# baegwangbin/MaGNet

Hardware: NVIDIA H100
Metric: frames/sec (640x480, 4 views, 64 hyp) (higher is better)
Workload: dtype f32

## Files before the change

### magnet_b200/csrc/api.cu

```cuda
#include <atomic>
#include <cstdlib>
#include <cstdio>
#include <cstring>

#include "common.cuh"

namespace magnet {
cudaError_t launch_cost_direct(const CostParams& p, int depth_mode, int src_layout, int C, bool cw,
                               bool softmax, cudaStream_t st, int* launches);
cudaError_t launch_cost_cells(const CostParams& p, int mode, int C, bool cw, bool reuse, cudaStream_t st);
cudaError_t launch_softmax_planes(float* vol, int B, int D, int HW, cudaStream_t st);
bool cells_supports(int C, int D, int layout);
cudaError_t launch_cost_tma(const CostParams& p, int mode, int C, bool cw, cudaStream_t st);
bool tma_supports(int C, int D, int V, int layout);
void tma_launch_info(int B, int H, int W, int D, int* grid, int* block, int* smem);
cudaError_t launch_cost_mma(const CostParams& p, int mode, bool cw, cudaStream_t st);
bool mma_supports(int C, int D, int V, int layout);
void mma_launch_info(int B, int H, int W, int D, int* grid, int* block, int* smem);
size_t split16_buffer_bytes(int N, int H, int W);
cudaError_t launch_repack_split16(const float* src, const float* gmm, void* dst, int N, int C, int H, int W,
                                  cudaStream_t st, int* launches);
#ifdef MAGNET_MMA_DEBUG
void mma_set_debug_buffer(float* p);
#endif
cudaError_t launch_repack_pixc(const float* src, const float* gmm, float* dst, int N, int C, int H, int W,
                               cudaStream_t st);
void cells_launch_info(int B, int H, int W, int D, int* grid, int* block, int* smem);
cudaError_t launch_pack_cameras(const float* intM, const float* R, int64_t r_sb, int64_t r_sv, int64_t r_si,
                                int64_t r_sj, const float* t, int64_t t_sb, int64_t t_sv, int64_t t_si,
                                const int32_t* is_valid, int B, int V, magnet_camera* out, cudaStream_t st);
cudaError_t launch_repack(const float* src, float* dst, int N, int C, int H, int W, cudaStream_t st);
cudaError_t launch_sample(const float* gmm, const float* k_host, int B, int D, int HW, float* dvol,
                          cudaStream_t st);
cudaError_t launch_update_fwd(const float* dout, const float* gmm0, int B, int HW, float* out, cudaStream_t st);
cudaError_t launch_update_bwd(const float* gout, const float* dout, const float* gmm0, int B, int HW, float* gin,
                              cudaStream_t st);
cudaError_t launch_relative_poses(const float* ext_ref, const float* ext_nghbr, int B, int V, float* poses,
                                  int32_t* valid, cudaStream_t st);
cudaError_t launch_camera_rays(const double* raw, int B, int H, int W, float* intM, float* rays, cudaStream_t st);
cudaError_t launch_upsample_fwd(const float* depth, const float* mask, int B, int CH, int H, int W, int k, float* out,
                                cudaStream_t st);
cudaError_t launch_upsample_bwd(const float* gout, const float* depth, const float* mask, int B, int CH, int H, int W,
                                int k, float* gdepth, float* gmask, cudaStream_t st);
cudaError_t launch_cost_f_bwd(const BwdParams& p, cudaStream_t st, int* launches);
cudaError_t launch_cost_f_bwd_mma(const BwdParams& p, cudaStream_t st, int* launches);
bool f_bwd_mma_supports(int C, int V);
cudaError_t launch_cost_cw_bwd(const CwBwdParams& p, const CwBwdParams* split, int C, int mode, bool mask_mma,
                               const float* grad_out, cudaStream_t st, int* launches);
bool cw_bwd_supports(int C);
#ifdef MAGNET_MMA_DEBUG
void f_bwd_mma_set_debug_buffer(float* p);
#endif
int fnet_l1_partials(int B, int HW);
cudaError_t launch_fnet_l1_fwd(const float* scores, const float* planes, const float* gt, const uint8_t* mask, int B,
                               int D, int HW, float* partial, cudaStream_t st);
cudaError_t launch_fnet_l1_bwd(const float* scores, const float* planes, const float* gt, const uint8_t* mask,
                               float scale, const float* grad_scale, int B, int D, int HW, float* grad_scores,
                               cudaStream_t st);
cudaError_t launch_upsample_nll_fwd(const float* depth, const float* mask, const float* gt, const uint8_t* gtm, int B,
                                    int H, int W, int k, float* partial, cudaStream_t st);
cudaError_t launch_upsample_nll_bwd(const float* depth, const float* mask, const float* gt, const uint8_t* gtm, float scale,
                                    int B, int H, int W, int k, float* gdepth, float* gmask, cudaStream_t st);
}

namespace {
std::atomic<uint64_t> g_launches{0};
thread_local char g_cuda_err[256] = "";

int cuda_fail(cudaError_t e) {
  snprintf(g_cuda_err, sizeof(g_cuda_err), "%s: %s", cudaGetErrorName(e), cudaGetErrorString(e));
  return MAGNET_ERR_CUDA;
}

int validate_cost(const magnet_cost_args* a) {
  if (!a) return MAGNET_ERR_NULL;
// ... 222 lines not shown
                            const int32_t* is_valid, int32_t B, int32_t V, magnet_camera* cams_out,
                            void* stream) {
  if (!intM || !R || !t || !is_valid || !cams_out) return MAGNET_ERR_NULL;
  if (B <= 0 || V <= 0) return MAGNET_ERR_SHAPE;
  cudaError_t e = magnet::launch_pack_cameras(intM, R, r_sb, r_sv, r_si, r_sj, t, t_sb, t_sv, t_si, is_valid, B, V,
                                              cams_out, (cudaStream_t)stream);
  if (e != cudaSuccess) return cuda_fail(e);
  g_launches += 1;
  return MAGNET_OK;
}

int magnet_repack_tiled32_f32(const float* src_nchw, float* dst, int32_t N, int32_t C, int32_t H, int32_t W,
                            void* stream) {
  if (!src_nchw || !dst) return MAGNET_ERR_NULL;
  if (N <= 0 || C <= 0 || H <= 0 || W <= 0) return MAGNET_ERR_SHAPE;
  if (C % 4 != 0 || C / 4 > 65535 || N > 65535) return MAGNET_ERR_UNSUPPORTED;
  if (reinterpret_cast<uintptr_t>(dst) % 16 != 0) return MAGNET_ERR_ALIGN;
  cudaError_t e = magnet::launch_repack(src_nchw, dst, N, C, H, W, (cudaStream_t)stream);
  if (e != cudaSuccess) return cuda_fail(e);
  g_launches += 1;
  return MAGNET_OK;
}

int magnet_repack_pixc_f32(const float* src_nchw, const float* src_gmm, float* dst, int32_t N, int32_t C, int32_t H,
                           int32_t W, void* stream) {
  if (!src_nchw || !dst) return MAGNET_ERR_NULL;
  if (N <= 0 || C <= 0 || H <= 0 || W <= 0 || N > 65535) return MAGNET_ERR_SHAPE;
  if (C != 16 && C != 32 && C != 64) return MAGNET_ERR_UNSUPPORTED;
  if (reinterpret_cast<uintptr_t>(dst) % 16 != 0) return MAGNET_ERR_ALIGN;
  cudaError_t e = magnet::launch_repack_pixc(src_nchw, src_gmm, dst, N, C, H, W, (cudaStream_t)stream);
  if (e != cudaSuccess) return cuda_fail(e);
  g_launches += 1;
  return MAGNET_OK;
}

size_t magnet_split16_bytes(int32_t N, int32_t H, int32_t W) {
  if (N <= 0 || H <= 0 || W <= 0) return 0;
  return magnet::split16_buffer_bytes(N, H, W);
}

int magnet_repack_split16_f32(const float* src_nchw, const float* src_gmm, void* dst, int32_t N, int32_t C, int32_t H,
                              int32_t W, void* stream) {
  if (!src_nchw || !dst) return MAGNET_ERR_NULL;
  if (N <= 0 || C <= 0 || H <= 0 || W <= 0 || N > 65535) return MAGNET_ERR_SHAPE;
  if (C != 64) return MAGNET_ERR_UNSUPPORTED;
  if (reinterpret_cast<uintptr_t>(dst) % 16 != 0 || reinterpret_cast<uintptr_t>(src_nchw) % 16 != 0) return MAGNET_ERR_ALIGN;
  int launches = 0;
  cudaError_t e = magnet::launch_repack_split16(src_nchw, src_gmm, dst, N, C, H, W, (cudaStream_t)stream, &launches);
  if (e != cudaSuccess) return cuda_fail(e);
  g_launches += launches;
  return MAGNET_OK;
}

#ifdef MAGNET_MMA_DEBUG
void magnet_mma_debug_buffer(float* p) { magnet::mma_set_debug_buffer(p); }
void magnet_f_bwd_mma_debug_buffer(float* p) { magnet::f_bwd_mma_set_debug_buffer(p); }
#endif

int magnet_sample_depths_f32(const float* gmm, const float* k_host, int32_t B, int32_t D, int32_t HW,
                             float* d_volume, void* stream) {
  if (!gmm || !k_host || !d_volume) return MAGNET_ERR_NULL;
  if (B <= 0 || D <= 0 || HW <= 0) return MAGNET_ERR_SHAPE;
  if (D > MAGNET_MAX_PLANES || B > 65535) return MAGNET_ERR_UNSUPPORTED;
  cudaError_t e = magnet::launch_sample(gmm, k_host, B, D, HW, d_volume, (cudaStream_t)stream);
  if (e != cudaSuccess) return cuda_fail(e);
  g_launches += 1;
  return MAGNET_OK;
}

int magnet_gaussian_update_fwd_f32(const float* d_output, const float* ref_gmm, int32_t B, int32_t HW,
                                   float* out, void* stream) {
  if (!d_output || !ref_gmm || !out) return MAGNET_ERR_NULL;
  if (B <= 0 || HW <= 0 || B > 65535) return MAGNET_ERR_SHAPE;
  cudaError_t e = magnet::launch_update_fwd(d_output, ref_gmm, B, HW, out, (cudaStream_t)stream);
  if (e != cudaSuccess) return cuda_fail(e);
  g_launches += 1;
  return MAGNET_OK;
}

int magnet_gaussian_update_bwd_f32(const float* grad_out, const float* d_output, const float* ref_gmm,
                                   int32_t B, int32_t HW, float* grad_d_output, void* stream) {
  if (!grad_out || !d_output || !ref_gmm || !grad_d_output) return MAGNET_ERR_NULL;
  if (B <= 0 || HW <= 0 || B > 65535) return MAGNET_ERR_SHAPE;
  cudaError_t e = magnet::launch_update_bwd(grad_out, d_output, ref_gmm, B, HW, grad_d_output, (cudaStream_t)stream);
  if (e != cudaSuccess) return cuda_fail(e);
  g_launches += 1;
  return MAGNET_OK;
}

int magnet_relative_poses_f32(const float* ext_ref, const float* ext_nghbr, int32_t B, int32_t V, float* poses_out,
                              int32_t* is_valid_out, void* stream) {
  if (!ext_ref || !ext_nghbr || !poses_out || !is_valid_out) return MAGNET_ERR_NULL;
  if (B <= 0 || V <= 0) return MAGNET_ERR_SHAPE;
  cudaError_t e = magnet::launch_relative_poses(ext_ref, ext_nghbr, B, V, poses_out, is_valid_out, (cudaStream_t)stream);
  if (e != cudaSuccess) return cuda_fail(e);
  g_launches += 1;
  return MAGNET_OK;
}

int magnet_camera_rays_f32(const double* raw_intrinsics, int32_t B, int32_t H, int32_t W, float* intM_out,
                           float* rays_out, void* stream) {
  if (!raw_intrinsics || !intM_out || !rays_out) return MAGNET_ERR_NULL;
  if (B <= 0 || H <= 0 || W <= 0 || B > 65535) return MAGNET_ERR_SHAPE;
  cudaError_t e = magnet::launch_camera_rays(raw_intrinsics, B, H, W, intM_out, rays_out, (cudaStream_t)stream);
  if (e != cudaSuccess) return cuda_fail(e);
  g_launches += 1;
  return MAGNET_OK;
}
// ... 94 lines not shown
```

### magnet_b200/csrc/cost_mma.cu

```cuda
#include <cuda_fp16.h>

#include <algorithm>
#include <atomic>
#include <cstddef>
#include <mutex>
#include <type_traits>

#include "common.cuh"
#include "tma_common.cuh"
#include "cw_mask.cuh"

namespace magnet {

constexpr int MNT = 256;
constexpr int MTW = 8, MTH = 8;
constexpr int MPX = MTW * MTH;
constexpr int MCH = 64;
constexpr int MSEG = 32;
constexpr int MMAXV = 16;
constexpr int SEG_BYTES = 2048;
constexpr int META_SEG_BYTES = 128;

constexpr int MOFF_A = 0;
constexpr int MOFF_R = 16384;
constexpr int MR_BYTES = 67584;
constexpr int MOFF_META = MOFF_R + MR_BYTES;
constexpr int MOFF_CAM = MOFF_META + MSEG * META_SEG_BYTES;
constexpr int MOFF_KS = MOFF_CAM + MMAXV * 64;
constexpr int MOFF_BBOX = MOFF_KS + MCH * 4;
constexpr int MOFF_BAR = MOFF_BBOX + 64;
constexpr int MOFF_ACC = MOFF_BAR + 64;
constexpr int MOFF_PIX = MOFF_ACC + MCH * 65 * 4;
constexpr int M_SMEM_USED = MOFF_PIX + 8 * 8 * 32;
constexpr int M_SMEM_TOTAL = M_SMEM_USED + 1024;
static_assert(MR_BYTES >= MSEG * SEG_BYTES && MR_BYTES >= MPX * 264 * 4 && MR_BYTES >= MCH * 65 * 4, "region R");
static_assert(2 * (M_SMEM_TOTAL + 1024) <= 227 * 1024, "two CTAs per SM");

__host__ __device__ inline size_t split16_bytes(size_t N, size_t H, size_t W) {
  return SPLIT16_HEADER + N * H * W * 256 + N * H * (W + 1) * 16;
}

constexpr int MMA_SLOTS = 1024;
__device__ unsigned g_mma_next[MMA_SLOTS];
__device__ unsigned g_mma_done[MMA_SLOTS];

__device__ __forceinline__ float lds_f32(uint32_t a) {
  float v;
  asm volatile("ld.shared.f32 %0, [%1];" : "=f"(v) : "r"(a));
  return v;
}
__device__ __forceinline__ float4 lds_f32x4(uint32_t a) {
  float4 v;
  asm volatile("ld.shared.v4.f32 {%0, %1, %2, %3}, [%4];" : "=f"(v.x), "=f"(v.y), "=f"(v.z), "=f"(v.w) : "r"(a));
  return v;
}
template <int MODE, bool CW>
__global__ void __launch_bounds__(MNT, 2)
cost_mma_kernel(const __grid_constant__ CostParams p, const __grid_constant__ CUtensorMap tm_ref,
                const __grid_constant__ CUtensorMap tm_src, const __grid_constant__ CUtensorMap tm_meta, const int nchunks,
                const int n_items, const int slot, float* __restrict__ dbg) {
  extern __shared__ unsigned char smem_raw[];
  const uint32_t raw = smem_u32(smem_raw);
  const uint32_t padb = (1024u - (raw & 1023u)) & 1023u;
  unsigned char* smem = smem_raw + padb;
  const uint32_t sbase = raw + padb;
  const magnet_camera* cams_s = reinterpret_cast<const magnet_camera*>(smem + MOFF_CAM);
  float* ks = reinterpret_cast<float*>(smem + MOFF_KS);
  int* bbox = reinterpret_cast<int*>(smem + MOFF_BBOX);
  float* regR = reinterpret_cast<float*>(smem + MOFF_R);
  const uint32_t bar_tma = sbase + MOFF_BAR, bar_cam = sbase + MOFF_BAR + 24;
  float* acc_s = reinterpret_cast<float*>(smem + MOFF_ACC);
  const unsigned FULL = 0xffffffffu;

  const int tid = threadIdx.x, lane = tid & 31, warp = tid >> 5;
  const int H = p.H, W = p.W, HW = p.HW, D = p.D, V = p.V;
  const int tiles_x = (W + MTW - 1) / MTW;
  const int items_per_b = tiles_x * ((H + MTH - 1) / MTH) * nchunks;

  const unsigned char* refbuf = reinterpret_cast<const unsigned char*>(p.ref_feat);
  const unsigned char* srcbuf = reinterpret_cast<const unsigned char*>(p.src_feat);
  const Split16Header* hdr_ref = reinterpret_cast<const Split16Header*>(refbuf);
  const Split16Header* hdr_src = reinterpret_cast<const Split16Header*>(srcbuf);
  volatile int* next_item = reinterpret_cast<volatile int*>(smem + MOFF_BAR + 40);

  if (tid == 0) {
    mbar_init(bar_tma, 1);
    mbar_init(bar_cam, 1);
    fence_mbar_init();
    prefetch_tmap(&tm_ref);
    prefetch_tmap(&tm_src);
    prefetch_tmap(&tm_meta);
  }
  if (tid < 8) bbox[tid] = (tid & 1) ? -(1 << 28) : (1 << 28);
  __syncthreads();
  uint32_t ph_tma = 0, ph_cam = 0;
  int it = 0;
  int cur_b = -1;
  const float xmax = (float)W + 1.0f, ymax = (float)H + 1.0f;
  const float kappa = p.kappa;
  const uint32_t g_row0 = sbase + MOFF_R, m_base = sbase + MOFF_META;

  int item = blockIdx.x;
  while (item < n_items) {
  const int b = item / items_per_b;
  const int rem = item - b * items_per_b;
  const int tile = rem / nchunks;
  const int jc = (rem - tile * nchunks) * MCH;
  const int Dc = min(MCH, D - jc);
  const int tx0 = (tile % tiles_x) * MTW, ty0 = (tile / tiles_x) * MTH;

  if (tid == 0) {
    if (b != cur_b) {
      mbar_arrive_expect_tx(bar_cam, (uint32_t)V * 64u);
      bulk_load(sbase + MOFF_CAM, p.cams + (size_t)b * V, (uint32_t)V * 64u, bar_cam);
    }
    tma_load_5d(sbase + MOFF_A, &tm_ref, bar_tma, 0, tx0, ty0, 0, b);
    *next_item = (int)gridDim.x + (int)atomicAdd(&g_mma_next[slot], 1u);
  }
  if (tid < MCH) ks[tid] = MODE != MAGNET_DEPTH_VOLUME ? p.k[min(jc + tid, D - 1)] : 0.0f;
  for (int idx = tid; idx < MCH * 65; idx += MNT) acc_s[idx] = 0.0f;
  __syncthreads();

  const int py = ty0 + warp;
  float R0, R1, R2, MU = 0.f, SG = 0.f;
  unsigned livemask;
  {
    const int px = tx0 + (lane & 7);
    const bool live = px < W && py < H;
    const int n = min(py, H - 1) * W + min(px, W - 1);
    R0 = ldg_f(p.rays + ((size_t)b * 3 + 0) * HW + n);
    R1 = ldg_f(p.rays + ((size_t)b * 3 + 1) * HW + n);
    R2 = ldg_f(p.rays + ((size_t)b * 3 + 2) * HW + n);
    if (MODE == MAGNET_DEPTH_GAUSS) {
      MU = ldg_f(p.ref_gmm + ((size_t)b * 2 + 0) * HW + n);
      SG = ldg_f(p.ref_gmm + ((size_t)b * 2 + 1) * HW + n);
    }
    livemask = __ballot_sync(FULL, live) & 0xffu;
  }
  float2 dvol[MODE == MAGNET_DEPTH_VOLUME ? MTW : 1];
  float2 k2 = make_float2(0.f, 0.f);
  if (MODE == MAGNET_DEPTH_VOLUME) {
    for (int idx = tid; idx < MCH * MPX; idx += MNT) {
      const int j = idx >> 6, pp = idx & 63;
      const int y = ty0 + (pp >> 3), x = tx0 + (pp & 7);
      const size_t n = (size_t)min(y, H - 1) * W + min(x, W - 1);
      regR[j * 65 + pp] = ldg_f(p.d_volume + ((size_t)b * D + jc + min(j, Dc - 1)) * HW + n);
    }
    __syncthreads();
#pragma unroll
    for (int i = 0; i < MTW; ++i) dvol[i] = make_float2(regR[lane * 65 + warp * 8 + i], regR[(lane + 32) * 65 + warp * 8 + i]);
    fence_proxy_async();
    __syncthreads();
  } else {
    k2 = make_float2(ks[lane], ks[lane + 32]);
  }
  auto depth2 = [&](const int i, const float mu, const float sg) -> float2 {
    if (MODE == MAGNET_DEPTH_VOLUME) return dvol[i];
    if (MODE == MAGNET_DEPTH_PLANES) return k2;
    return fadd2_rn(make_float2(mu, mu), make_float2(__fmul_rn(sg, k2.x), __fmul_rn(sg, k2.y)));
  };
  float4* pixt = reinterpret_cast<float4*>(smem + MOFF_PIX) + warp * 16;

  if (b != cur_b) {
    mbar_wait_or_trap(bar_cam, ph_cam);
    ph_cam ^= 1u;
    cur_b = b;
  }
  bool first = true;

  for (int v = 0; v < V; ++v) {
    const magnet_camera* cam = cams_s + v;
    if (cam->valid != 1.0f) continue;
    const float a0 = cam->a[0], a1 = cam->a[1], a2 = cam->a[2];
    const float Q0 = __fmaf_rn(cam->A[2], R2, __fmaf_rn(cam->A[1], R1, __fmul_rn(cam->A[0], R0)));
    const float Q1 = __fmaf_rn(cam->A[5], R2, __fmaf_rn(cam->A[4], R1, __fmul_rn(cam->A[3], R0)));
    const float Q2 = __fmaf_rn(cam->A[8], R2, __fmaf_rn(cam->A[7], R1, __fmul_rn(cam->A[6], R0)));
    __syncwarp();
    if (lane < 8) {
      pixt[2 * lane] = make_float4(Q0, Q1, Q2, 0.0f);
      pixt[2 * lane + 1] = make_float4(Q2, MU, SG, 0.0f);
    }
    __syncwarp();
    const int vb = v * p.B + b;
    auto project_px = [&](const int i, float2& ix, float2& iy, float2& z) {
      const float4 t1 = pixt[2 * i], t2 = pixt[2 * i + 1];
      project2(depth2(i, t2.y, t2.z), a0, a1, a2, t1.x, t1.y, t1.z, ix, iy, z);
      ix.x = clamp_coord(ix.x, xmax); ix.y = clamp_coord(ix.y, xmax);
      iy.x = clamp_coord(iy.x, ymax); iy.y = clamp_coord(iy.y, ymax);
    };

    float xl = 1e9f, xh = -1e9f, yl = 1e9f, yh = -1e9f;
#pragma unroll
    for (int i = 0; i < MTW; ++i) {
      float2 ix, iy, z;
      project_px(i, ix, iy, z);
      if ((livemask >> i) & 1u) {
        xl = fminf(xl, fminf(ix.x, ix.y)); xh = fmaxf(xh, fmaxf(ix.x, ix.y));
        yl = fminf(yl, fminf(iy.x, iy.y)); yh = fmaxf(yh, fmaxf(iy.x, iy.y));
      }
    }
    int* bb = bbox + (it & 1) * 4;
    {
      const int r0 = __reduce_min_sync(FULL, (int)floorf(xl)), r1 = __reduce_max_sync(FULL, (int)floorf(xh));
      const int r2 = __reduce_min_sync(FULL, (int)floorf(yl)), r3 = __reduce_max_sync(FULL, (int)floorf(yh));
      if (lane == 0) { atomicMin(bb + 0, r0); atomicMax(bb + 1, r1); atomicMin(bb + 2, r2); atomicMax(bb + 3, r3); }
    }
    fence_proxy_async();
    __syncthreads();
    const int wx0 = bb[0], wx1 = bb[1], wy0 = bb[2], wy1 = bb[3];
    if (tid < 4) bbox[((it + 1) & 1) * 4 + tid] = (tid & 1) ? -(1 << 28) : (1 << 28);
    ++it;
    const int nseg_all = (wx1 - wx0 + 2 + 7) >> 3, rows_all = wy1 - wy0 + 2;
    const int nsw = min(nseg_all, 16);
    const int rmax = nseg_all * rows_all <= MSEG ? rows_all : max(2, MSEG / nsw);
    const int stepx = 8 * nsw - 1, stepy = rmax - 1;

    for (int sy = wy0; sy <= wy1; sy += stepy) {
      const int rows = min(stepy, wy1 - sy + 1) + 1;
      for (int sx = wx0; sx <= wx1; sx += stepx) {
        const int nseg = (min(stepx, wx1 - sx + 1) + 1 + 7) >> 3;
        const int nsegs = nseg * rows;
        if (tid == 0)
          mbar_arrive_expect_tx(bar_tma, (uint32_t)nsegs * (SEG_BYTES + (CW ? META_SEG_BYTES : 0)) + (first ? 16384u : 0u));
        first = false;
        if (lane == 0) {
          for (int s = warp; s < nsegs; s += MNT / 32) {
            const int r = s / nseg, xb = s - r * nseg;
            tma_load_5d(sbase + MOFF_R + (uint32_t)s * SEG_BYTES, &tm_src, bar_tma, 0, sx + 8 * xb, sy + r, 0, vb);
            if (CW) tma_load_4d(m_base + (uint32_t)s * META_SEG_BYTES, &tm_meta, bar_tma, 0, sx + 8 * xb + 1, sy + r, vb);
          }
        }
        __syncwarp();
        const int npad = (nsegs * 8 + 15) & ~15;
        const int gp = ((npad + 23) & ~31) + 8;
        mbar_wait_or_trap(bar_tma, ph_tma);
        ph_tma ^= 1u;
        {
          const int wg = warp >> 2;
          float acc[64];
#pragma unroll
          for (int e = 0; e < 64; ++e) acc[e] = 0.0f;
          const uint32_t bseg = sbase + MOFF_R + (uint32_t)(wg * 16 * SEG_BYTES);
          const uint64_t a_hi = gmma_desc_sw128(sbase + MOFF_A, 1024), a_lo = gmma_desc_sw128(sbase + MOFF_A + 8192, 1024);
          const uint64_t b_hi = gmma_desc_sw128(bseg, SEG_BYTES), b_lo = gmma_desc_sw128(bseg + 1024, SEG_BYTES);
          __syncwarp();
          if (wg == 0 || npad > 128) {
            wgmma_fence();
#pragma unroll
            for (int pr = 0; pr < 3; ++pr) {
              const uint64_t ad = pr == 0 ? a_lo : a_hi, bd = pr == 1 ? b_lo : b_hi;
#pragma unroll
              for (int kk = 0; kk < 4; ++kk) wgmma_m64n128k16_f16(acc, ad + 2u * kk, bd + 2u * kk, (pr | kk) != 0);
            }
            wgmma_commit();
            wgmma_wait_all();
          }
          __syncthreads();
          const int r0 = ((warp & 3) << 4) + (lane >> 2);
          float* g0 = regR + (size_t)r0 * gp + wg * 128 + 2 * (lane & 3);
#pragma unroll
          for (int j = 0; j < 16; ++j) {
            if (wg * 128 + 8 * j < npad) {
              *reinterpret_cast<float2*>(g0 + 8 * j) = make_float2(acc[4 * j], acc[4 * j + 1]);
              *reinterpret_cast<float2*>(g0 + 8 * gp + 8 * j) = make_float2(acc[4 * j + 2], acc[4 * j + 3]);
            }
          }
          __syncthreads();
        }
#ifdef MAGNET_MMA_DEBUG
        if (dbg != nullptr && item == 0 && v == 0 && sy == wy0 && sx == wx0) {
          if (tid == 0) {
            dbg[0] = (float)sx; dbg[1] = (float)sy; dbg[2] = (float)nseg; dbg[3] = (float)rows; dbg[4] = (float)npad;
            dbg[5] = (float)gp; dbg[6] = (float)v; dbg[7] = 3.0f; dbg[8] = hdr_ref->scale; dbg[9] = hdr_src->scale;
          }
          for (int idx = tid; idx < MPX * npad; idx += MNT) dbg[16 + (idx / npad) * 256 + idx % npad] = regR[(idx / npad) * gp + idx % npad];
        }
#endif
        const bool single = nseg_all * rows_all <= MSEG;
        auto phase_c = [&](auto single_tag) {
          constexpr bool SINGLE = decltype(single_tag)::value;
          const float MAGIC = 12582912.0f;
          const float sxf = (float)sx, syf = (float)sy;
          const float xend = sx + stepx > wx1 ? 1e9f : (float)(sx + stepx), yend = sy + stepy > wy1 ? 1e9f : (float)(sy + stepy);
          const float pitch4f = (float)(nseg * 32);
          const float c0f = MAGIC - 4.0f * sxf - pitch4f * syf;
          const uint32_t pitch4 = (uint32_t)nseg * 32u;
          uint32_t rowaddr = g_row0 + (uint32_t)(warp * 8 * gp) * 4u;
          float* accp = acc_s + lane * 65 + warp * 8;
#pragma unroll
          for (int i = 0; i < MTW; ++i, rowaddr += (uint32_t)gp * 4u) {
            if (!((livemask >> i) & 1u)) continue;
            float2 x, y, z;
            project_px(i, x, y, z);
            float2 x0, y0, fx, fy;
            cell_split(x.x, x0.x, fx.x); cell_split(x.y, x0.y, fx.y);
            cell_split(y.x, y0.x, fy.x); cell_split(y.y, y0.y, fy.y);
            const float2 m1 = make_float2(-1.0f, -1.0f);
            const float2 o = ffma2_rn(y0, make_float2(pitch4f, pitch4f), ffma2_rn(x0, make_float2(4.0f, 4.0f), make_float2(c0f, c0f)));
            uint32_t ca = __float_as_uint(o.x) & 0x3fffffu, cb = __float_as_uint(o.y) & 0x3fffffu;
            bool pa = true, pb = true;
            if (!SINGLE) {
              pa = x0.x >= sxf && x0.x < xend && y0.x >= syf && y0.x < yend;
              pb = x0.y >= sxf && x0.y < xend && y0.y >= syf && y0.y < yend;
              ca = pa ? ca : 0u;
              cb = pb ? cb : 0u;
            }
            const uint32_t ga = rowaddr + ca, gb = rowaddr + cb;
            const float2 g00 = make_float2(lds_f32(ga), lds_f32(gb)), g01 = make_float2(lds_f32(ga + 4), lds_f32(gb + 4));
            const float2 g10 = make_float2(lds_f32(ga + pitch4), lds_f32(gb + pitch4));
            const float2 g11 = make_float2(lds_f32(ga + pitch4 + 4), lds_f32(gb + pitch4 + 4));
            const float2 ct = ffma2_rn(fx, ffma2_rn(g00, m1, g01), g00), cu = ffma2_rn(fx, ffma2_rn(g10, m1, g11), g10);
            const float2 cost = ffma2_rn(fy, ffma2_rn(ct, m1, cu), ct);
            const float costa = cost.x, costb = cost.y;
            bool oka, okb;
            if (CW) {
              const uint32_t ma = m_base + ca * 4u, mb = m_base + cb * 4u;
              const float2 msa = lerp2d_x2(lds_f32x4(ma), lds_f32x4(ma + pitch4 * 4u), fx.x, fy.x);
              const float2 msb = lerp2d_x2(lds_f32x4(mb), lds_f32x4(mb + pitch4 * 4u), fx.y, fy.y);
              oka = cw_keep(z.x, msa, kappa);
              okb = cw_keep(z.y, msb, kappa);
            } else {
              oka = fabsf(costa) < 3.0e38f;
              okb = fabsf(costb) < 3.0e38f;
            }
            if (pa && oka) accp[i] += costa;
            if (pb && okb) accp[32 * 65 + i] += costb;
          }
        };
        if (single) phase_c(std::true_type{});
        else phase_c(std::false_type{});
        fence_proxy_async();
        __syncthreads();
      }
    }
  }

  if (first) {
    if (tid == 0) mbar_arrive_expect_tx(bar_tma, 16384u);
    mbar_wait_or_trap(bar_tma, ph_tma);
    ph_tma ^= 1u;
  }

  {
    const float inv = hdr_ref->inv_scale * hdr_src->inv_scale;
    const bool exact = p.inv_v_exact != 0.0f;
    auto fin = [&](float a) { a *= inv; return exact ? a * p.inv_v_exact : __fdiv_rn(a, p.vf); };
    if ((W & 3) == 0 && (reinterpret_cast<uintptr_t>(p.out) & 15) == 0) {
      for (int idx = tid; idx < MCH * 16; idx += MNT) {
        const int j = idx >> 4, r = (idx >> 1) & 7, hx = (idx & 1) * 4;
        const int y = ty0 + r, x = tx0 + hx;
        if (j < Dc && x < W && y < H) {
          const float* a = acc_s + j * 65 + r * 8 + hx;
          *reinterpret_cast<float4*>(p.out + ((size_t)b * D + jc + j) * HW + (size_t)y * W + x) =
              make_float4(fin(a[0]), fin(a[1]), fin(a[2]), fin(a[3]));
        }
      }
    } else {
      for (int idx = tid; idx < MCH * MPX; idx += MNT) {
        const int j = idx >> 6, pp = idx & 63;
        const int y = ty0 + (pp >> 3), x = tx0 + (pp & 7);
        if (j < Dc && x < W && y < H) p.out[((size_t)b * D + jc + j) * HW + (size_t)y * W + x] = fin(acc_s[j * 65 + pp]);
      }
    }
  }
  const int nxt = *next_item;
  __syncthreads();
  item = nxt;
  }

  if (tid == 0) {
    __threadfence();
    if (atomicAdd(&g_mma_done[slot], 1u) == gridDim.x - 1) {
      g_mma_next[slot] = 0u;
      g_mma_done[slot] = 0u;
      __threadfence();
    }
  }
}

__device__ __forceinline__ unsigned finite_abs_bits(float x) {
  const unsigned u = __float_as_uint(x) & 0x7fffffffu;
  return u >= 0x7f800000u ? 0u : u;
}

__global__ void __launch_bounds__(256) absmax_kernel(const float4* __restrict__ x, size_t n4, const float* __restrict__ tail,
                                                     int ntail, unsigned* __restrict__ out) {
  unsigned m = 0u;
  for (size_t i = (size_t)blockIdx.x * blockDim.x + threadIdx.x; i < n4; i += (size_t)gridDim.x * blockDim.x) {
    const float4 v = __ldg(x + i);
    m = max(max(m, finite_abs_bits(v.x)), finite_abs_bits(v.y));
    m = max(max(m, finite_abs_bits(v.z)), finite_abs_bits(v.w));
  }
  if (blockIdx.x == 0 && (int)threadIdx.x < ntail) m = max(m, finite_abs_bits(tail[threadIdx.x]));
  m = __reduce_max_sync(0xffffffffu, m);
  if ((threadIdx.x & 31) == 0 && m != 0u) atomicMax(out, m);
}

__device__ __forceinline__ int split16_shift(unsigned absmax_bits) {
  const int e = (int)(absmax_bits >> 23) & 0xff;
  if (e == 0 || e == 255) return 0;
  return max(-100, min(100, 14 - (e - 127)));
}

template <int SPX, bool VEC>
__global__ void __launch_bounds__(256) split16_repack_kernel(const float* __restrict__ src, const float* __restrict__ gmm,
                                                             unsigned char* __restrict__ dst, int N, int HW, int W) {
  constexpr int C = 64;
  __shared__ float t[SPX * (C + 1)];
  Split16Header* hdr = reinterpret_cast<Split16Header*>(dst);
  const int sh = split16_shift(hdr->absmax);
  const float s = __uint_as_float((unsigned)(127 + sh) << 23);
  if (blockIdx.x == 0 && blockIdx.y == 0 && threadIdx.x == 0) {
    hdr->scale = s;
    hdr->inv_scale = __uint_as_float((unsigned)(127 - sh) << 23);
  }
  const size_t img = blockIdx.y;
  const int p0 = blockIdx.x * SPX;
  if constexpr (VEC) {
    static_assert(SPX == 128, "thread mapping below");
    constexpr int CPI = 8;
    const int lane = threadIdx.x & 31, warp = threadIdx.x >> 5;
    const int q4 = (warp & 3) * 8 + (lane & 7), c0 = (warp >> 2) * 4 + (lane >> 3);
// ... 65 lines not shown
  const int HW = H * W;
  const size_t n = (size_t)N * C * HW;
  cudaError_t e = cudaMemsetAsync(dst, 0, SPLIT16_HEADER, st);
  if (e != cudaSuccess) return e;
  const size_t n4 = n / 4;
  int dev = 0;
  if ((e = cudaGetDevice(&dev)) != cudaSuccess) return e;
  const int blocks = (int)std::min<size_t>((size_t)sm_count(dev) * 8, (n4 + 255) / 256 + 1);
  absmax_kernel<<<blocks, 256, 0, st>>>(reinterpret_cast<const float4*>(src), n4, src + n4 * 4, (int)(n - n4 * 4),
                                        reinterpret_cast<unsigned*>(static_cast<unsigned char*>(dst) + offsetof(Split16Header, absmax)));
  dim3 block(256);
  if (HW % 4 == 0 && reinterpret_cast<uintptr_t>(src) % 16 == 0) {
    dim3 grid((HW + 127) / 128, N);
    split16_repack_kernel<128, true><<<grid, block, 0, st>>>(src, gmm, static_cast<unsigned char*>(dst), N, HW, W);
  } else {
    dim3 grid((HW + 31) / 32, N);
    split16_repack_kernel<32, false><<<grid, block, 0, st>>>(src, gmm, static_cast<unsigned char*>(dst), N, HW, W);
  }
  *launches = 2;
  return cudaGetLastError();
}

typedef CUresult (*EncodeTiledFn)(CUtensorMap*, CUtensorMapDataType, cuuint32_t, void*, const cuuint64_t*,
                                  const cuuint64_t*, const cuuint32_t*, const cuuint32_t*, CUtensorMapInterleave,
                                  CUtensorMapSwizzle, CUtensorMapL2promotion, CUtensorMapFloatOOBfill);
EncodeTiledFn encode_tiled_fn();

cudaError_t make_planes_map(CUtensorMap* tm, const void* planes, int N, int H, int W, int box_rows) {
  EncodeTiledFn enc = encode_tiled_fn();
  if (!enc) return cudaErrorNotSupported;
  const cuuint64_t dims[5] = {64, (cuuint64_t)W, (cuuint64_t)H, 2, (cuuint64_t)N};
  const cuuint64_t strides[4] = {128, (cuuint64_t)W * 128, (cuuint64_t)H * W * 128, (cuuint64_t)H * W * 256};
  const cuuint32_t box[5] = {64u, 8u, (cuuint32_t)box_rows, 2u, 1u};
  const cuuint32_t estr[5] = {1u, 1u, 1u, 1u, 1u};
  const CUresult r = enc(tm, CU_TENSOR_MAP_DATA_TYPE_FLOAT16, 5, const_cast<void*>(planes), dims, strides, box, estr,
                         CU_TENSOR_MAP_INTERLEAVE_NONE, CU_TENSOR_MAP_SWIZZLE_128B, CU_TENSOR_MAP_L2_PROMOTION_L2_256B,
                         CU_TENSOR_MAP_FLOAT_OOB_FILL_NONE);
  return r == CUDA_SUCCESS ? cudaSuccess : cudaErrorInvalidValue;
}

static cudaError_t make_meta_map(CUtensorMap* tm, const void* meta, int N, int H, int W) {
  EncodeTiledFn enc = encode_tiled_fn();
  if (!enc) return cudaErrorNotSupported;
  const cuuint64_t dims[4] = {4, (cuuint64_t)W + 1, (cuuint64_t)H, (cuuint64_t)N};
  const cuuint64_t strides[3] = {16, ((cuuint64_t)W + 1) * 16, (cuuint64_t)H * (W + 1) * 16};
  const cuuint32_t box[4] = {4u, 8u, 1u, 1u};
  const cuuint32_t estr[4] = {1u, 1u, 1u, 1u};
  const CUresult r = enc(tm, CU_TENSOR_MAP_DATA_TYPE_FLOAT32, 4, const_cast<void*>(meta), dims, strides, box, estr,
                         CU_TENSOR_MAP_INTERLEAVE_NONE, CU_TENSOR_MAP_SWIZZLE_NONE, CU_TENSOR_MAP_L2_PROMOTION_L2_128B,
                         CU_TENSOR_MAP_FLOAT_OOB_FILL_NONE);
  return r == CUDA_SUCCESS ? cudaSuccess : cudaErrorInvalidValue;
}

#ifdef MAGNET_MMA_DEBUG
static float* g_mma_dbg = nullptr;
void mma_set_debug_buffer(float* p) { g_mma_dbg = p; }
#endif

template <int MODE, bool CW>
static cudaError_t launch_mma_mw(const CostParams& p, cudaStream_t st) {
  static std::once_flag flags[64];
  auto kern = cost_mma_kernel<MODE, CW>;
  int dev = 0;
  cudaError_t e = cudaGetDevice(&dev);
  if (e != cudaSuccess) return e;
  cudaError_t res = cudaSuccess;
  std::call_once(flags[dev & 63], [&] {
    res = cudaFuncSetAttribute(kern, cudaFuncAttributeMaxDynamicSharedMemorySize, M_SMEM_TOTAL);
    if (res == cudaSuccess)
      res = cudaFuncSetAttribute(kern, cudaFuncAttributePreferredSharedMemoryCarveout, cudaSharedmemCarveoutMaxShared);
  });
  if (res != cudaSuccess) return res;
  const int N = p.B * p.V;
  const unsigned char* refbuf = reinterpret_cast<const unsigned char*>(p.ref_feat);
  const unsigned char* srcbuf = reinterpret_cast<const unsigned char*>(p.src_feat);
  CUtensorMap tm_ref, tm_src, tm_meta;
  if ((e = make_planes_map(&tm_ref, refbuf + SPLIT16_HEADER, p.B, p.H, p.W, 8)) != cudaSuccess) return e;
  if ((e = make_planes_map(&tm_src, srcbuf + SPLIT16_HEADER, N, p.H, p.W, 1)) != cudaSuccess) return e;
  if ((e = make_meta_map(&tm_meta, srcbuf + SPLIT16_HEADER + (size_t)N * p.HW * 256, N, p.H, p.W)) != cudaSuccess) return e;
  const int nchunks = (p.D + MCH - 1) / MCH;
  const int tiles = ((p.W + MTW - 1) / MTW) * ((p.H + MTH - 1) / MTH);
  const int n_items = tiles * nchunks * p.B;
  static std::atomic<unsigned> ticket{0}, graph_ticket{0};
  cudaStreamCaptureStatus cap = cudaStreamCaptureStatusNone;
  if (cudaStreamIsCapturing(st, &cap) != cudaSuccess) cap = cudaStreamCaptureStatusNone;
  const int slot = cap == cudaStreamCaptureStatusActive ? MMA_SLOTS / 2 + (int)(graph_ticket.fetch_add(1) % (MMA_SLOTS / 2))
                                                        : (int)(ticket.fetch_add(1) % (MMA_SLOTS / 2));
  dim3 grid(std::min(n_items, 2 * sm_count(dev))), block(MNT);
  float* dbg = nullptr;
#ifdef MAGNET_MMA_DEBUG
  dbg = g_mma_dbg;
#endif
  kern<<<grid, block, M_SMEM_TOTAL, st>>>(p, tm_ref, tm_src, tm_meta, nchunks, n_items, slot, dbg);
  return cudaGetLastError();
}

bool mma_supports(int C, int D, int V, int layout) {
  return C == 64 && layout == MAGNET_SRC_SPLIT16 && D >= 1 && V <= MMAXV;
}

void mma_launch_info(int B, int H, int W, int D, int* grid, int* block, int* smem) {
  int dev = 0;
  cudaGetDevice(&dev);
  *grid = std::min(((W + MTW - 1) / MTW) * ((H + MTH - 1) / MTH) * ((D + MCH - 1) / MCH) * B, 2 * sm_count(dev));
  *block = MNT;
  *smem = M_SMEM_TOTAL;
}

size_t split16_buffer_bytes(int N, int H, int W) { return split16_bytes((size_t)N, (size_t)H, (size_t)W); }

cudaError_t launch_cost_mma(const CostParams& p, int mode, bool cw, cudaStream_t st) {
  if (cw) {
    if (mode == MAGNET_DEPTH_VOLUME) return launch_mma_mw<MAGNET_DEPTH_VOLUME, true>(p, st);
    if (mode == MAGNET_DEPTH_GAUSS) return launch_mma_mw<MAGNET_DEPTH_GAUSS, true>(p, st);
    return launch_mma_mw<MAGNET_DEPTH_PLANES, true>(p, st);
  }
  if (mode == MAGNET_DEPTH_VOLUME) return launch_mma_mw<MAGNET_DEPTH_VOLUME, false>(p, st);
  if (mode == MAGNET_DEPTH_GAUSS) return launch_mma_mw<MAGNET_DEPTH_GAUSS, false>(p, st);
  return launch_mma_mw<MAGNET_DEPTH_PLANES, false>(p, st);
}

}
```

Baseline: 6089.

## Compute per-view window boxes analytically and overlap with phase C; keep accumulators in registers

Replaces the per-view bounding-box pass, which projected all eight pixels per warp, with an analytic two-endpoint projection over the depth range. It falls back to per-pixel projection only when the fast bound is unsafe. The box for the next valid view is now computed after the MMA stage of the current window, removing a block-wide sync per view. Cost accumulators move from shared memory into registers and are spilled to shared memory only in the epilogue, and depth-volume values are staged once into a padded shared buffer. It also adds optional clock64 stage profiling behind a compile flag, at the cost of more registers and a more complex ordering of barriers.

```diff
diff --git a/magnet_b200/csrc/api.cu b/magnet_b200/csrc/api.cu
--- a/magnet_b200/csrc/api.cu
+++ b/magnet_b200/csrc/api.cu
@@ -20,7 +20,7 @@
 size_t split16_buffer_bytes(int N, int H, int W);
 cudaError_t launch_repack_split16(const float* src, const float* gmm, void* dst, int N, int C, int H, int W,
                                   cudaStream_t st, int* launches);
-#ifdef MAGNET_MMA_DEBUG
+#if defined(MAGNET_MMA_DEBUG) || defined(MAGNET_MMA_PROFILE)
 void mma_set_debug_buffer(float* p);
 #endif
 cudaError_t launch_repack_pixc(const float* src, const float* gmm, float* dst, int N, int C, int H, int W,
@@ -349,8 +349,10 @@
   return MAGNET_OK;
 }
 
+#if defined(MAGNET_MMA_DEBUG) || defined(MAGNET_MMA_PROFILE)
+void magnet_mma_debug_buffer(float* p) { magnet::mma_set_debug_buffer(p); }
+#endif
 #ifdef MAGNET_MMA_DEBUG
-void magnet_mma_debug_buffer(float* p) { magnet::mma_set_debug_buffer(p); }
 void magnet_f_bwd_mma_debug_buffer(float* p) { magnet::f_bwd_mma_set_debug_buffer(p); }
 #endif
 
diff --git a/magnet_b200/csrc/cost_mma.cu b/magnet_b200/csrc/cost_mma.cu
--- a/magnet_b200/csrc/cost_mma.cu
+++ b/magnet_b200/csrc/cost_mma.cu
@@ -29,11 +29,14 @@
 constexpr int MOFF_KS = MOFF_CAM + MMAXV * 64;
 constexpr int MOFF_BBOX = MOFF_KS + MCH * 4;
 constexpr int MOFF_BAR = MOFF_BBOX + 64;
-constexpr int MOFF_ACC = MOFF_BAR + 64;
-constexpr int MOFF_PIX = MOFF_ACC + MCH * 65 * 4;
+constexpr int MOFF_DV = MOFF_BAR + 64;
+constexpr int MOFF_DEND = MOFF_DV + MPX * 65 * 4;
+constexpr int MOFF_PIXR = MOFF_DEND + MPX * 8;
+constexpr int MOFF_PIX = MOFF_PIXR + MPX * 32;
 constexpr int M_SMEM_USED = MOFF_PIX + 8 * 8 * 32;
 constexpr int M_SMEM_TOTAL = M_SMEM_USED + 1024;
 static_assert(MR_BYTES >= MSEG * SEG_BYTES && MR_BYTES >= MPX * 264 * 4 && MR_BYTES >= MCH * 65 * 4, "region R");
+constexpr int MMA_DBG_OUTSIDE = 16 + MPX * 256;
 static_assert(2 * (M_SMEM_TOTAL + 1024) <= 227 * 1024, "two CTAs per SM");
 
 __host__ __device__ inline size_t split16_bytes(size_t N, size_t H, size_t W) {
@@ -54,6 +57,20 @@
   asm volatile("ld.shared.v4.f32 {%0, %1, %2, %3}, [%4];" : "=f"(v.x), "=f"(v.y), "=f"(v.z), "=f"(v.w) : "r"(a));
   return v;
 }
+enum { PROF_SETUP, PROF_BOX, PROF_TMA, PROF_MMA, PROF_PHASEC, PROF_EPI, PROF_NSTAGES };
+#ifdef MAGNET_MMA_PROFILE
+#define MMA_STAGE(s)                                                                                                   \
+  do {                                                                                                                 \
+    if (tid == 0) {                                                                                                    \
+      const long long t_ = clock64();                                                                                  \
+      prof_s[s] += t_ - prof_s[7];                                                                                     \
+      prof_s[7] = t_;                                                                                                  \
+    }                                                                                                                  \
+  } while (0)
+#else
+#define MMA_STAGE(s) do { } while (0)
+#endif
+
 template <int MODE, bool CW>
 __global__ void __launch_bounds__(MNT, 2)
 cost_mma_kernel(const __grid_constant__ CostParams p, const __grid_constant__ CUtensorMap tm_ref,
@@ -69,10 +86,13 @@
   int* bbox = reinterpret_cast<int*>(smem + MOFF_BBOX);
   float* regR = reinterpret_cast<float*>(smem + MOFF_R);
   const uint32_t bar_tma = sbase + MOFF_BAR, bar_cam = sbase + MOFF_BAR + 24;
-  float* acc_s = reinterpret_cast<float*>(smem + MOFF_ACC);
   const unsigned FULL = 0xffffffffu;
 
   const int tid = threadIdx.x, lane = tid & 31, warp = tid >> 5;
+#ifdef MAGNET_MMA_PROFILE
+  __shared__ long long prof_s[8];
+  if (tid < 8) prof_s[tid] = tid == 7 ? clock64() : 0ll;
+#endif
   const int H = p.H, W = p.W, HW = p.HW, D = p.D, V = p.V;
   const int tiles_x = (W + MTW - 1) / MTW;
   const int items_per_b = tiles_x * ((H + MTH - 1) / MTH) * nchunks;
@@ -98,6 +118,8 @@
   int cur_b = -1;
   const float xmax = (float)W + 1.0f, ymax = (float)H + 1.0f;
   const float kappa = p.kappa;
+  constexpr float BOX_EPS = 0.015625f;
+  const float amp_max = 65536.0f / (float)(max(W, H) + 3) - 8.0f;
   const uint32_t g_row0 = sbase + MOFF_R, m_base = sbase + MOFF_META;
 
   int item = blockIdx.x;
@@ -118,13 +140,13 @@
     *next_item = (int)gridDim.x + (int)atomicAdd(&g_mma_next[slot], 1u);
   }
   if (tid < MCH) ks[tid] = MODE != MAGNET_DEPTH_VOLUME ? p.k[min(jc + tid, D - 1)] : 0.0f;
-  for (int idx = tid; idx < MCH * 65; idx += MNT) acc_s[idx] = 0.0f;
   __syncthreads();
 
   const int py = ty0 + warp;
-  float R0, R1, R2, MU = 0.f, SG = 0.f;
+  float4* pixr = reinterpret_cast<float4*>(smem + MOFF_PIXR) + warp * 16;
   unsigned livemask;
   {
+    float R0, R1, R2, MU = 0.f, SG = 0.f;
     const int px = tx0 + (lane & 7);
     const bool live = px < W && py < H;
     const int n = min(py, H - 1) * W + min(px, W - 1);
@@ -136,77 +158,138 @@
       SG = ldg_f(p.ref_gmm + ((size_t)b * 2 + 1) * HW + n);
     }
     livemask = __ballot_sync(FULL, live) & 0xffu;
-  }
-  float2 dvol[MODE == MAGNET_DEPTH_VOLUME ? MTW : 1];
-  float2 k2 = make_float2(0.f, 0.f);
+    if (lane < 8) {
+      pixr[2 * lane] = make_float4(R0, R1, R2, 0.0f);
+      pixr[2 * lane + 1] = make_float4(MU, SG, 0.0f, 0.0f);
+    }
+    __syncwarp();
+  }
+  const uint32_t dvw = sbase + MOFF_DV + (uint32_t)(warp * 8 * 65 + lane) * 4u;
   if (MODE == MAGNET_DEPTH_VOLUME) {
-    for (int idx = tid; idx < MCH * MPX; idx += MNT) {
-      const int j = idx >> 6, pp = idx & 63;
-      const int y = ty0 + (pp >> 3), x = tx0 + (pp & 7);
-      const size_t n = (size_t)min(y, H - 1) * W + min(x, W - 1);
-      regR[j * 65 + pp] = ldg_f(p.d_volume + ((size_t)b * D + jc + min(j, Dc - 1)) * HW + n);
+    float* dv_s = reinterpret_cast<float*>(smem + MOFF_DV);
+    const int pp = tid & 63, y = ty0 + (pp >> 3), x = tx0 + (pp & 7);
+    const float* dsrc = p.d_volume + ((size_t)b * D + jc) * HW + (size_t)min(y, H - 1) * W + min(x, W - 1);
+#pragma unroll 1
+    for (int j0 = tid >> 6; j0 < MCH; j0 += 32) {
+      float dl[8];
+#pragma unroll
+      for (int r = 0; r < 8; ++r) dl[r] = ldg_f(dsrc + (size_t)min(j0 + 4 * r, Dc - 1) * HW);
+#pragma unroll
+      for (int r = 0; r < 8; ++r) dv_s[pp * 65 + j0 + 4 * r] = dl[r];
     }
     __syncthreads();
 #pragma unroll
-    for (int i = 0; i < MTW; ++i) dvol[i] = make_float2(regR[lane * 65 + warp * 8 + i], regR[(lane + 32) * 65 + warp * 8 + i]);
-    fence_proxy_async();
-    __syncthreads();
-  } else {
-    k2 = make_float2(ks[lane], ks[lane + 32]);
+    for (int i = 0; i < MTW; ++i) {
+      const float da = lds_f32(dvw + i * 260), db = lds_f32(dvw + i * 260 + 128);
+      float lo = fminf(da, db), hi = fmaxf(da, db);
+      const bool fin = __all_sync(FULL, isfinite(da) && isfinite(db));
+#pragma unroll
+      for (int o = 16; o > 0; o >>= 1) {
+        lo = fminf(lo, __shfl_xor_sync(FULL, lo, o));
+        hi = fmaxf(hi, __shfl_xor_sync(FULL, hi, o));
+      }
+      if (lane == i) reinterpret_cast<float2*>(smem + MOFF_DEND)[warp * 8 + i] = fin ? make_float2(lo, hi) : make_float2(NAN, NAN);
+    }
+    __syncwarp();
   }
   auto depth2 = [&](const int i, const float mu, const float sg) -> float2 {
-    if (MODE == MAGNET_DEPTH_VOLUME) return dvol[i];
+    if (MODE == MAGNET_DEPTH_VOLUME) return make_float2(lds_f32(dvw + i * 260), lds_f32(dvw + i * 260 + 128));
+    const float2 k2 = make_float2(ks[lane], ks[lane + 32]);
     if (MODE == MAGNET_DEPTH_PLANES) return k2;
     return fadd2_rn(make_float2(mu, mu), make_float2(__fmul_rn(sg, k2.x), __fmul_rn(sg, k2.y)));
   };
   float4* pixt = reinterpret_cast<float4*>(smem + MOFF_PIX) + warp * 16;
 
+  auto window_box = [&](const int v, int* bb) {
+    const magnet_camera* cam = cams_s + v;
+    const float a0 = cam->a[0], a1 = cam->a[1], a2 = cam->a[2];
+    const float4 ray = pixr[2 * (lane & 7)];
+    const float MU = pixr[2 * (lane & 7) + 1].x, SG = pixr[2 * (lane & 7) + 1].y;
+    const float Q0 = __fmaf_rn(cam->A[2], ray.z, __fmaf_rn(cam->A[1], ray.y, __fmul_rn(cam->A[0], ray.x)));
+    const float Q1 = __fmaf_rn(cam->A[5], ray.z, __fmaf_rn(cam->A[4], ray.y, __fmul_rn(cam->A[3], ray.x)));
+    const float Q2 = __fmaf_rn(cam->A[8], ray.z, __fmaf_rn(cam->A[7], ray.y, __fmul_rn(cam->A[6], ray.x)));
+    float2 dr;
+    if (MODE == MAGNET_DEPTH_VOLUME) {
+      const uint32_t a = sbase + MOFF_DEND + (uint32_t)(warp * 8 + (lane & 7)) * 8u;
+      dr = make_float2(lds_f32(a), lds_f32(a + 4));
+    }
+    else if (MODE == MAGNET_DEPTH_PLANES) dr = make_float2(ks[0], ks[MCH - 1]);
+    else dr = fadd2_rn(make_float2(MU, MU), make_float2(__fmul_rn(SG, ks[0]), __fmul_rn(SG, ks[MCH - 1])));
+    float2 ix, iy, z;
+    project2(dr, a0, a1, a2, Q0, Q1, Q2, ix, iy, z);
+    const float amp = fmaxf(fabsf(__fmul_rn(Q2, dr.x)) / z.x, fabsf(__fmul_rn(Q2, dr.y)) / z.y) + 2.0e-3f / fminf(z.x, z.y);
+    const bool ok = (MODE == MAGNET_DEPTH_VOLUME || p.k_sorted) && isfinite(dr.x) && isfinite(dr.y) && z.x > 0.0f &&
+                    z.y > 0.0f && amp <= amp_max && isfinite(ix.x) && isfinite(ix.y) && isfinite(iy.x) && isfinite(iy.y);
+    const bool live = (livemask >> (lane & 7)) & 1u;
+    float xl = 1e9f, xh = -1e9f, yl = 1e9f, yh = -1e9f;
+    if (__all_sync(FULL, ok || !live)) {
+      if (live) {
+        xl = clamp_coord(__fsub_rn(fminf(ix.x, ix.y), BOX_EPS), xmax); xh = clamp_coord(__fadd_rn(fmaxf(ix.x, ix.y), BOX_EPS), xmax);
+        yl = clamp_coord(__fsub_rn(fminf(iy.x, iy.y), BOX_EPS), ymax); yh = clamp_coord(__fadd_rn(fmaxf(iy.x, iy.y), BOX_EPS), ymax);
+      }
+    } else {
+#ifdef MAGNET_MMA_DEBUG
+      if (dbg != nullptr && lane == 0) atomicAdd(reinterpret_cast<unsigned*>(dbg + MMA_DBG_OUTSIDE + 1), 1u);
+#endif
+#pragma unroll
+      for (int i = 0; i < MTW; ++i) {
+        const float q0 = __shfl_sync(FULL, Q0, i), q1 = __shfl_sync(FULL, Q1, i), q2 = __shfl_sync(FULL, Q2, i);
+        const float mu = __shfl_sync(FULL, MU, i), sg = __shfl_sync(FULL, SG, i);
+        project2(depth2(i, mu, sg), a0, a1, a2, q0, q1, q2, ix, iy, z);
+        ix.x = clamp_coord(ix.x, xmax); ix.y = clamp_coord(ix.y, xmax);
+        iy.x = clamp_coord(iy.x, ymax); iy.y = clamp_coord(iy.y, ymax);
+        if ((livemask >> i) & 1u) {
+          xl = fminf(xl, fminf(ix.x, ix.y)); xh = fmaxf(xh, fmaxf(ix.x, ix.y));
+          yl = fminf(yl, fminf(iy.x, iy.y)); yh = fmaxf(yh, fmaxf(iy.x, iy.y));
+        }
+      }
+    }
+    const int r0 = __reduce_min_sync(FULL, (int)floorf(xl)), r1 = __reduce_max_sync(FULL, (int)floorf(xh));
+    const int r2 = __reduce_min_sync(FULL, (int)floorf(yl)), r3 = __reduce_max_sync(FULL, (int)floorf(yh));
+    if (lane == 0) { atomicMin(bb + 0, r0); atomicMax(bb + 1, r1); atomicMin(bb + 2, r2); atomicMax(bb + 3, r3); }
+  };
+  auto next_valid = [&](int v) {
+    while (v < V && cams_s[v].valid != 1.0f) ++v;
+    return v;
+  };
+
   if (b != cur_b) {
     mbar_wait_or_trap(bar_cam, ph_cam);
     ph_cam ^= 1u;
     cur_b = b;
   }
   bool first = true;
-
-  for (int v = 0; v < V; ++v) {
-    const magnet_camera* cam = cams_s + v;
-    if (cam->valid != 1.0f) continue;
-    const float a0 = cam->a[0], a1 = cam->a[1], a2 = cam->a[2];
-    const float Q0 = __fmaf_rn(cam->A[2], R2, __fmaf_rn(cam->A[1], R1, __fmul_rn(cam->A[0], R0)));
-    const float Q1 = __fmaf_rn(cam->A[5], R2, __fmaf_rn(cam->A[4], R1, __fmul_rn(cam->A[3], R0)));
-    const float Q2 = __fmaf_rn(cam->A[8], R2, __fmaf_rn(cam->A[7], R1, __fmul_rn(cam->A[6], R0)));
+  float2 accr[MTW];
+#pragma unroll
+  for (int i = 0; i < MTW; ++i) accr[i] = make_float2(0.0f, 0.0f);
+  MMA_STAGE(PROF_SETUP);
+  int v = next_valid(0);
+  if (v < V) window_box(v, bbox + (it & 1) * 4);
+  __syncthreads();
+  MMA_STAGE(PROF_BOX);
+
+  while (v < V) {
+    const int vn = next_valid(v + 1);
     __syncwarp();
     if (lane < 8) {
-      pixt[2 * lane] = make_float4(Q0, Q1, Q2, 0.0f);
-      pixt[2 * lane + 1] = make_float4(Q2, MU, SG, 0.0f);
+      const magnet_camera* cam = cams_s + v;
+      const float4 ray = pixr[2 * lane], ms = pixr[2 * lane + 1];
+      const float Q0 = __fmaf_rn(cam->A[2], ray.z, __fmaf_rn(cam->A[1], ray.y, __fmul_rn(cam->A[0], ray.x)));
+      const float Q1 = __fmaf_rn(cam->A[5], ray.z, __fmaf_rn(cam->A[4], ray.y, __fmul_rn(cam->A[3], ray.x)));
+      const float Q2 = __fmaf_rn(cam->A[8], ray.z, __fmaf_rn(cam->A[7], ray.y, __fmul_rn(cam->A[6], ray.x)));
+      pixt[2 * lane] = make_float4(Q0, Q1, Q2, cam->a[0]);
+      pixt[2 * lane + 1] = make_float4(cam->a[1], ms.x, ms.y, cam->a[2]);
     }
     __syncwarp();
     const int vb = v * p.B + b;
     auto project_px = [&](const int i, float2& ix, float2& iy, float2& z) {
       const float4 t1 = pixt[2 * i], t2 = pixt[2 * i + 1];
-      project2(depth2(i, t2.y, t2.z), a0, a1, a2, t1.x, t1.y, t1.z, ix, iy, z);
+      project2(depth2(i, t2.y, t2.z), t1.w, t2.x, t2.w, t1.x, t1.y, t1.z, ix, iy, z);
       ix.x = clamp_coord(ix.x, xmax); ix.y = clamp_coord(ix.y, xmax);
       iy.x = clamp_coord(iy.x, ymax); iy.y = clamp_coord(iy.y, ymax);
     };
 
-    float xl = 1e9f, xh = -1e9f, yl = 1e9f, yh = -1e9f;
-#pragma unroll
-    for (int i = 0; i < MTW; ++i) {
-      float2 ix, iy, z;
-      project_px(i, ix, iy, z);
-      if ((livemask >> i) & 1u) {
-        xl = fminf(xl, fminf(ix.x, ix.y)); xh = fmaxf(xh, fmaxf(ix.x, ix.y));
-        yl = fminf(yl, fminf(iy.x, iy.y)); yh = fmaxf(yh, fmaxf(iy.x, iy.y));
-      }
-    }
-    int* bb = bbox + (it & 1) * 4;
-    {
-      const int r0 = __reduce_min_sync(FULL, (int)floorf(xl)), r1 = __reduce_max_sync(FULL, (int)floorf(xh));
-      const int r2 = __reduce_min_sync(FULL, (int)floorf(yl)), r3 = __reduce_max_sync(FULL, (int)floorf(yh));
-      if (lane == 0) { atomicMin(bb + 0, r0); atomicMax(bb + 1, r1); atomicMin(bb + 2, r2); atomicMax(bb + 3, r3); }
-    }
-    fence_proxy_async();
-    __syncthreads();
+    const int* bb = bbox + (it & 1) * 4;
     const int wx0 = bb[0], wx1 = bb[1], wy0 = bb[2], wy1 = bb[3];
     if (tid < 4) bbox[((it + 1) & 1) * 4 + tid] = (tid & 1) ? -(1 << 28) : (1 << 28);
     ++it;
@@ -235,6 +318,7 @@
         const int gp = ((npad + 23) & ~31) + 8;
         mbar_wait_or_trap(bar_tma, ph_tma);
         ph_tma ^= 1u;
+        MMA_STAGE(PROF_TMA);
         {
           const int wg = warp >> 2;
           float acc[64];
@@ -267,6 +351,7 @@
           }
           __syncthreads();
         }
+        MMA_STAGE(PROF_MMA);
 #ifdef MAGNET_MMA_DEBUG
         if (dbg != nullptr && item == 0 && v == 0 && sy == wy0 && sx == wx0) {
           if (tid == 0) {
@@ -276,6 +361,8 @@
           for (int idx = tid; idx < MPX * npad; idx += MNT) dbg[16 + (idx / npad) * 256 + idx % npad] = regR[(idx / npad) * gp + idx % npad];
         }
 #endif
+        if (sy == wy0 && sx == wx0 && vn < V) window_box(vn, bbox + (it & 1) * 4);
+        MMA_STAGE(PROF_BOX);
         const bool single = nseg_all * rows_all <= MSEG;
         auto phase_c = [&](auto single_tag) {
           constexpr bool SINGLE = decltype(single_tag)::value;
@@ -286,7 +373,7 @@
           const float c0f = MAGIC - 4.0f * sxf - pitch4f * syf;
           const uint32_t pitch4 = (uint32_t)nseg * 32u;
           uint32_t rowaddr = g_row0 + (uint32_t)(warp * 8 * gp) * 4u;
-          float* accp = acc_s + lane * 65 + warp * 8;
+          const uint32_t cmax = pitch4 * (uint32_t)(rows - 1) - 8u;
 #pragma unroll
           for (int i = 0; i < MTW; ++i, rowaddr += (uint32_t)gp * 4u) {
             if (!((livemask >> i) & 1u)) continue;
@@ -304,7 +391,18 @@
               pb = x0.y >= sxf && x0.y < xend && y0.y >= syf && y0.y < yend;
               ca = pa ? ca : 0u;
               cb = pb ? cb : 0u;
+            } else {
+              ca = min(ca, cmax);
+              cb = min(cb, cmax);
             }
+#ifdef MAGNET_MMA_DEBUG
+            if (dbg != nullptr && sy == wy0 && sx == wx0) {
+              const bool outa = lane < Dc && (x0.x < (float)wx0 || x0.x > (float)wx1 || y0.x < (float)wy0 || y0.x > (float)wy1);
+              const bool outb = lane + 32 < Dc && (x0.y < (float)wx0 || x0.y > (float)wx1 || y0.y < (float)wy0 || y0.y > (float)wy1);
+              const unsigned nout = __popc(__ballot_sync(FULL, outa)) + __popc(__ballot_sync(FULL, outb));
+              if (lane == 0 && nout != 0u) atomicAdd(reinterpret_cast<unsigned*>(dbg + MMA_DBG_OUTSIDE), nout);
+            }
+#endif
             const uint32_t ga = rowaddr + ca, gb = rowaddr + cb;
             const float2 g00 = make_float2(lds_f32(ga), lds_f32(gb)), g01 = make_float2(lds_f32(ga + 4), lds_f32(gb + 4));
             const float2 g10 = make_float2(lds_f32(ga + pitch4), lds_f32(gb + pitch4));
@@ -323,16 +421,18 @@
               oka = fabsf(costa) < 3.0e38f;
               okb = fabsf(costb) < 3.0e38f;
             }
-            if (pa && oka) accp[i] += costa;
-            if (pb && okb) accp[32 * 65 + i] += costb;
+            if (pa && oka) accr[i].x += costa;
+            if (pb && okb) accr[i].y += costb;
           }
         };
         if (single) phase_c(std::true_type{});
         else phase_c(std::false_type{});
         fence_proxy_async();
         __syncthreads();
+        MMA_STAGE(PROF_PHASEC);
       }
     }
+    v = vn;
   }
 
   if (first) {
@@ -342,6 +442,19 @@
   }
 
   {
+    float* acc_s = regR;
+    const int b = item / items_per_b;
+    const int rem = item - b * items_per_b;
+    const int tile = rem / nchunks;
+    const int jc = (rem - tile * nchunks) * MCH;
+    const int Dc = min(MCH, D - jc);
+    const int tx0 = (tile % tiles_x) * MTW, ty0 = (tile / tiles_x) * MTH;
+#pragma unroll
+    for (int i = 0; i < MTW; ++i) {
+      acc_s[lane * 65 + warp * 8 + i] = accr[i].x;
+      acc_s[(lane + 32) * 65 + warp * 8 + i] = accr[i].y;
+    }
+    __syncthreads();
     const float inv = hdr_ref->inv_scale * hdr_src->inv_scale;
     const bool exact = p.inv_v_exact != 0.0f;
     auto fin = [&](float a) { a *= inv; return exact ? a * p.inv_v_exact : __fdiv_rn(a, p.vf); };
@@ -364,10 +477,19 @@
     }
   }
   const int nxt = *next_item;
+  fence_proxy_async();
   __syncthreads();
+  MMA_STAGE(PROF_EPI);
   item = nxt;
   }
 
+#ifdef MAGNET_MMA_PROFILE
+  if (tid == 0 && dbg != nullptr) {
+    unsigned long long* tot = reinterpret_cast<unsigned long long*>(dbg);
+    for (int s = 0; s < PROF_NSTAGES; ++s) atomicAdd(tot + s, (unsigned long long)prof_s[s]);
+    atomicAdd(tot + 7, 1ull);
+  }
+#endif
   if (tid == 0) {
     __threadfence();
     if (atomicAdd(&g_mma_done[slot], 1u) == gridDim.x - 1) {
@@ -539,7 +661,7 @@
   return r == CUDA_SUCCESS ? cudaSuccess : cudaErrorInvalidValue;
 }
 
-#ifdef MAGNET_MMA_DEBUG
+#if defined(MAGNET_MMA_DEBUG) || defined(MAGNET_MMA_PROFILE)
 static float* g_mma_dbg = nullptr;
 void mma_set_debug_buffer(float* p) { g_mma_dbg = p; }
 #endif
@@ -575,7 +697,7 @@
                                                         : (int)(ticket.fetch_add(1) % (MMA_SLOTS / 2));
   dim3 grid(std::min(n_items, 2 * sm_count(dev))), block(MNT);
   float* dbg = nullptr;
-#ifdef MAGNET_MMA_DEBUG
+#if defined(MAGNET_MMA_DEBUG) || defined(MAGNET_MMA_PROFILE)
   dbg = g_mma_dbg;
 #endif
   kern<<<grid, block, M_SMEM_TOTAL, st>>>(p, tm_ref, tm_src, tm_meta, nchunks, n_items, slot, dbg);
```

New measurement: 6439 (median of 6 runs). +5.8%, better.
